# sapeirone/EgoPack

Hardware: AMD Instinct MI355X
Metric: clip-seqs/sec training, AR+LTA+PNR multi-task (higher is better)
Workload: dtype bf16; 1 GPU; MTL pre-train AR+LTA+PNR (BASELINE config 3): per GPU B=64 seqs/task x T=32 nodes, 3x1536-d Omnivore-shaped features, H=1024, TRN hidden 1024 (dropout 0.5), depth 3, k=1, Adam; graph mode, fused backbone pass; global_batch=192, parallelism=dp1, trainable_params=25003272, capture=one graph, input=resident in HBM before the timed region, master_weights=f32, mode=bf16, activations=bf16

## Files before the change

### egopack_amd/csrc/gemm.hip

```cpp
#include <type_traits>

#include "common.h"

namespace egk {

typedef __attribute__((ext_vector_type(4))) float f32x4;
typedef __attribute__((ext_vector_type(8))) __bf16 bf16x8;
typedef unsigned short bf16_t;

constexpr int BM = 128, BN = 128, ROWB = 128;
constexpr int NTHREADS = 256;

constexpr int MAXSRC = 6;
struct GemmArgs {
    int M, N;
    int nsrc;
    int K[MAXSRC];
    const void* A[MAXSRC];
    const void* B[MAXSRC];
    long long lda[MAXSRC], ldb[MAXSRC];
    int a_vec, b_vec;
    void* C;
    long long ldc;
    int c_vec, c_bf16;
// ... 13 lines not shown
    int st_mode, st_nseg;
    const int* st_seg_ptr;
    double* st_ws;
    const void* st_x;
    long long st_ldx;
    const float* st_stats;
    const float* st_w;
    const float* st_b;
    float st_slope;
};

__device__ __forceinline__ void tile_of_virtual(const GemmArgs& g, int v, int& z, int& tm, int& tn) {
    const int tiles = g.tiles_m * g.tiles_n;
    z = v / tiles;
    const int t = v - z * tiles;
    const int gsz = g.group_m * g.tiles_n;
    const int grp = t / gsz, first = grp * g.group_m;
    const int rows = min(g.group_m, g.tiles_m - first);
    const int rr = t - grp * gsz;
    tm = first + rr % rows;
    tn = rr / rows;
}
__device__ __forceinline__ void tile_of(const GemmArgs& g, int bid, int& z, int& tm, int& tn) {
    const int tiles = g.tiles_m * g.tiles_n, nwg = tiles * g.splitk;
    const int xcd = bid & 7, q = nwg >> 3, r = nwg & 7;
    const int v = (xcd < r ? xcd * (q + 1) : r * (q + 1) + (xcd - r) * q) + (bid >> 3);
    z = v / tiles;
    const int t = v - z * tiles;
    const int gsz = g.group_m * g.tiles_n;
    const int grp = t / gsz, first = grp * g.group_m;
    const int rows = min(g.group_m, g.tiles_m - first);
    const int rr = t - grp * gsz;
    tm = first + rr % rows;
    tn = rr / rows;
}

template <int KT>
__device__ __forceinline__ void source_of(const GemmArgs& g, int t, int& src, int& tt) {
    src = 0;
    tt = t;
    while (src + 1 < g.nsrc) {
        const int n = (g.K[src] + KT - 1) / KT;
        if (tt < n) break;
        tt -= n;
        ++src;
    }
}
__device__ __forceinline__ int total_tiles(const GemmArgs& g, int KT) {
    int n = 0;
    for (int s = 0; s < g.nsrc; ++s) n += (g.K[s] + KT - 1) / KT;
    return n;
}

__device__ __forceinline__ int lds_off(int row, int chunk) { return row * ROWB + ((chunk ^ ((row >> 1) & 7)) << 4); }

__device__ __forceinline__ uint4 pack8(const float* f) {
    bf16x8 v;
#pragma unroll
    for (int i = 0; i < 8; ++i) v[i] = (__bf16)f[i];
    return __builtin_bit_cast(uint4, v);
}
__device__ __forceinline__ float bf16_to_f32(bf16_t h) { return __uint_as_float((unsigned)h << 16); }
__device__ __forceinline__ bf16_t f32_to_bf16(float f) { return __builtin_bit_cast(bf16_t, (__bf16)f); }


template <bool BF16C, typename T>
__device__ __forceinline__ void load_rowmajor(const T* __restrict__ base, long long ld, int rows_total, int row0, int k0,
                                              int klim, bool vec, uint4 (&out)[8]) {
    constexpr int CE = BF16C ? 8 : 4;
    const int tid = threadIdx.x;
#pragma unroll
    for (int i = 0; i < 4; ++i) {
        const int id = tid + NTHREADS * i;
        const int r = id >> 3, c = id & 7;
        const int grow = row0 + r, gk = k0 + c * CE;
        const bool row_ok = grow < rows_total;
        const T* p = base + (long long)grow * ld + gk;
        if constexpr (sizeof(T) == 2) {
            if (row_ok && vec && gk + 8 <= klim) out[i] = *reinterpret_cast<const uint4*>(p);
            else {
                unsigned w[4] = {0, 0, 0, 0};
#pragma unroll
                for (int j = 0; j < 8; ++j)
                    if (row_ok && gk + j < klim) w[j >> 1] |= (unsigned)p[j] << (16 * (j & 1));
                out[i] = make_uint4(w[0], w[1], w[2], w[3]);
            }
        } else {
            float f[8];
            if (row_ok && vec && gk + CE <= klim) {
                const float4 v0 = *reinterpret_cast<const float4*>(p);
                f[0] = v0.x; f[1] = v0.y; f[2] = v0.z; f[3] = v0.w;
                if constexpr (BF16C) {
                    const float4 v1 = *reinterpret_cast<const float4*>(p + 4);
                    f[4] = v1.x; f[5] = v1.y; f[6] = v1.z; f[7] = v1.w;
                }
            } else {
#pragma unroll
                for (int j = 0; j < CE; ++j) f[j] = (row_ok && gk + j < klim) ? p[j] : 0.0f;
            }
            if constexpr (BF16C) out[i] = pack8(f);
            else out[i] = make_uint4(__float_as_uint(f[0]), __float_as_uint(f[1]), __float_as_uint(f[2]), __float_as_uint(f[3]));
        }
    }
}

template <bool BF16C>
// ... 445 lines not shown
        const int piece = (first + i) & 15, sub_row0 = row0 + ((first + i) >> 4) * 128;
        if constexpr (TR) {
            const int k = piece * 4 + (lane >> 4);
            const int c = (lane & 15) ^ (2 * (k & 3) + 8 * ((k >> 3) & 1));
            int col = sub_row0 + c * 8;
            if (col + 8 > ld) col = 0;
            p[i] = base + (long long)(k0 + k) * ld + col;
        } else {
            const int r = piece * 8 + (lane >> 3);
            const int c = (lane & 7) ^ ((r >> 1) & 7);
            p[i] = base + (long long)min(sub_row0 + r, rows_total - 1) * ld + k0 + c * 8;
        }
    }
    step = (TR ? 64 * ld : 64) * tiles_per_step;
}
template <int NP, int OFF = 0, int TOT = NP>
__device__ __forceinline__ void cursor_issue(const bf16_t* (&pp)[TOT], long long step, unsigned char* img, int first) {
    const bf16_t** p = pp + OFF;
#pragma unroll
    for (int i = 0; i < NP; ++i) {
        __builtin_amdgcn_global_load_lds((glb_void_t*)p[i], (lds_void_t*)(img + (first + i) * 1024), 16, 0, 0);
        p[i] += step;
    }
}
template <bool TR, int NP>
struct OperandCursor {
    const bf16_t* p[NP];
    long long step;
    __device__ __forceinline__ void init(const bf16_t* __restrict__ base, long long ld, int rows_total, int row0, int k0,
                                         int first, int lane, int tiles_per_step) {
        cursor_init<TR, NP, 0, NP>(p, step, base, ld, rows_total, row0, k0, first, lane, tiles_per_step);
    }
    __device__ __forceinline__ void issue(unsigned char* img, int first) { cursor_issue<NP, 0, NP>(p, step, img, first); }
};

typedef _Float16 f16x8 __attribute__((ext_vector_type(8)));
template <bool F16>
__device__ __forceinline__ f32x4 mfma16(const uint4& b, const uint4& a, const f32x4& c) {
    if constexpr (F16) return __builtin_amdgcn_mfma_f32_16x16x32_f16(__builtin_bit_cast(f16x8, b), __builtin_bit_cast(f16x8, a), c, 0, 0, 0);
    else return __builtin_amdgcn_mfma_f32_16x16x32_bf16(__builtin_bit_cast(bf16x8, b), __builtin_bit_cast(bf16x8, a), c, 0, 0, 0);
}

template <int NSTAGE, bool TRA, bool TRB, int KG, int MB, int NI = 4, bool VIRT = false, bool F16 = false, int LW = 0>
__device__ __forceinline__ void gemm_pipe_body(const GemmArgs& g, const int bid) {
    static_assert(KG == 1 || MB == 1, "wave groups and the tall tile are alternatives");
    static_assert(NI == 4 || ((NI == 3 || NI == 2) && !TRA && ((MB == 1 && (KG == 1 || NI == 2)) || (MB == 2 && KG == 1 && NI == 3))),
                  "96- / 64-row tiles: row-major A; two wave groups with 64-row tiles only; the tall 8-wave tile with NI = 3");
    constexpr int IMG = 16384, IMG_A = NI == 4 ? MB * IMG : MB * NI * 4096, STAGE = IMG_A + IMG;
    constexpr int NPB = 4 / MB;
    constexpr int LOADS = NI + NPB;
    constexpr int WG = 4 * MB;
    extern __shared__ __attribute__((aligned(16))) unsigned char lds[];
    constexpr int KT = 64;
#ifdef EGK_GEMM_STAMPS
    const unsigned long long ps_entry = __builtin_amdgcn_s_memtime(), ps_rentry = __builtin_amdgcn_s_memrealtime();
    unsigned long long ps_first = 0;
#endif

    int z, tm, tn;
    if constexpr (VIRT) tile_of_virtual(g, bid, z, tm, tn);
    else tile_of(g, bid, z, tm, tn);
    const int m0 = tm * (32 * NI * MB), n0 = tn * BN;
    const int nkt = total_tiles(g, KT);
    const int per = (nkt + g.splitk - 1) / g.splitk;
    const int t_begin = z * per, t_end = min(nkt, t_begin + per);

    const int tid = threadIdx.x, lane = tid & 63;
    const int wall = __builtin_amdgcn_readfirstlane(tid >> 6);
    const int grp = KG == 1 ? 0 : (wall / WG);
    const int w = wall % WG;
    const int wm = w >> 1, wn = w & 1;
    const int lr = lane & 15, lg = lane >> 4;
    unsigned char* ring = lds + grp * (NSTAGE * STAGE);

    const int nt_all = t_end - t_begin;
    const int nt = nt_all > grp ? (nt_all - grp + KG - 1) / KG : 0;
    const int rounds = (nt_all + KG - 1) / KG;

    OperandCursor<TRA, NI> ca;
    OperandCursor<TRB, NPB> cb;
    int cur_src = -1;
    auto issue = [&](int i, int stage) {
        const int t = t_begin + grp + KG * i;
        int src, tt;
        source_of<KT>(g, t, src, tt);
        if (src != cur_src) {
            const int k0 = tt * KT;
            ca.init((const bf16_t*)g.A[src], g.lda[src], g.M, m0, k0, w * NI, lane, KG);
            cb.init((const bf16_t*)g.B[src], g.ldb[src], g.N, n0, k0, w * NPB, lane, KG);
            cur_src = src;
        }
        unsigned char* sbase = ring + stage * STAGE;
        ca.issue(sbase, w * NI);
        cb.issue(sbase + IMG_A, w * NPB);
    };

    if constexpr (LW > 0) {
        static_assert(KG == 1 && (WG * NI) % LW == 0 && (WG * NPB) % LW == 0, "loader waves: one wave group, pieces divisible among the loaders");
        if (wall >= WG) {
            constexpr int PA = WG * NI / LW, PB = WG * NPB / LW;
            const int L = wall - WG;
            OperandCursor<TRA, PA> la;
            OperandCursor<TRB, PB> lb;
            int lsrc = -1;
            auto lissue = [&](int i, int stage) {
                const int t = t_begin + i;
                int src, tt;
                source_of<KT>(g, t, src, tt);
                if (src != lsrc) {
                    const int k0 = tt * KT;
                    la.init((const bf16_t*)g.A[src], g.lda[src], g.M, m0, k0, L * PA, lane, 1);
                    lb.init((const bf16_t*)g.B[src], g.ldb[src], g.N, n0, k0, L * PB, lane, 1);
                    lsrc = src;
                }
                unsigned char* sbase = ring + stage * STAGE;
                la.issue(sbase, L * PA);
                lb.issue(sbase + IMG_A, L * PB);
            };
#pragma unroll
            for (int p = 0; p < NSTAGE - 1; ++p)
                if (p < nt) lissue(p, p);
            for (int it = 0; it < rounds; ++it) {
                const int later = min(NSTAGE - 2, nt - 1 - it);
                if (later >= 2) asm volatile("s_waitcnt vmcnt(%0)" ::"n"(2 * (PA + PB)) : "memory");
                else if (later == 1) asm volatile("s_waitcnt vmcnt(%0)" ::"n"(PA + PB) : "memory");
                else asm volatile("s_waitcnt vmcnt(0)" ::: "memory");
                __builtin_amdgcn_s_barrier();
                if (it + NSTAGE - 1 < nt) lissue(it + NSTAGE - 1, (it + NSTAGE - 1) % NSTAGE);
            }
            return;
        }
    }

    f32x4 acc[NI][4];
#pragma unroll
    for (int i = 0; i < NI; ++i)
#pragma unroll
        for (int j = 0; j < 4; ++j) acc[i][j] = f32x4{0.f, 0.f, 0.f, 0.f};

    const unsigned lds_base = (unsigned)(size_t)(lds_void_t*)ring;
    const unsigned rm_sw = (unsigned)((lg ^ ((lr >> 1) & 7)) << 4);
    const unsigned a_rm = (unsigned)((wm * 16 * NI + lr) * ROWB) + rm_sw;
    const unsigned b_rm = (unsigned)((wn * 64 + lr) * ROWB) + rm_sw;
    const int tq = (lane & 15) >> 2, tp = lane & 3;
    const unsigned tr_row = (unsigned)((8 * lg + tq) * 256 + (tp & 1) * 8);
    const unsigned tr_f = (unsigned)(2 * tq + 8 * (lg & 1));
    unsigned a_tr[4], b_tr[4];
#pragma unroll
    for (int i = 0; i < 4; ++i) {
        a_tr[i] = (unsigned)((wm >> 1) * IMG) + tr_row + ((((unsigned)((wm & 1) * 8 + 2 * i + (tp >> 1))) ^ tr_f) << 4);
        b_tr[i] = tr_row + ((((unsigned)(wn * 8 + 2 * i + (tp >> 1))) ^ tr_f) << 4);
    }

    const bool do_bias = TRA && g.dbias != nullptr && tn == 0;
    float bsum[8] = {0.f, 0.f, 0.f, 0.f, 0.f, 0.f, 0.f, 0.f};
    const int bcc = tid & 15, bkg = (tid & 255) >> 4;
    const int bsub = MB == 2 ? (tid >> 8) : 0;

    uint4 a0[4], a1[4], b0[4], b1[4];
    if constexpr (LW == 0) {
#pragma unroll
        for (int p = 0; p < NSTAGE - 1; ++p)
            if (p < nt) issue(p, p);
    }
    for (int it = 0; it < rounds; ++it) {
        if constexpr (LW == 0) {
            const int later = min(NSTAGE - 2, nt - 1 - it);
            if (later >= 3) asm volatile("s_waitcnt vmcnt(%0)" ::"n"(3 * LOADS) : "memory");
            else if (later == 2) asm volatile("s_waitcnt vmcnt(%0)" ::"n"(2 * LOADS) : "memory");
            else if (later == 1) asm volatile("s_waitcnt vmcnt(%0)" ::"n"(LOADS) : "memory");
            else asm volatile("s_waitcnt vmcnt(0)" ::: "memory");
        }
        __builtin_amdgcn_s_barrier();
#ifdef EGK_GEMM_STAMPS
        if (it == 0) ps_first = __builtin_amdgcn_s_memtime();
#endif
        const unsigned stA = lds_base + (it % NSTAGE) * STAGE, stB = stA + IMG_A;
        if constexpr (LW == 0) {
            if (it + NSTAGE - 1 < nt) issue(it + NSTAGE - 1, (it + NSTAGE - 1) % NSTAGE);
        }
        if (KG > 1 && it >= nt) continue;

        uint4 bz[4];
        if constexpr (TRA) {
            if (do_bias) {
#pragma unroll
                for (int r = 0; r < 4; ++r) {
                    const int k = bkg * 4 + r;
                    const unsigned ad = stA + (unsigned)(bsub * IMG + k * 256 + ((bcc ^ (2 * (k & 3) + 8 * ((k >> 3) & 1))) << 4));
                    asm volatile("ds_read_b128 %0, %1" : "=v"(bz[r]) : "v"(ad));
                }
            }
        }
        if constexpr (TRA) {
#pragma unroll
            for (int i = 0; i < 4; ++i) {
                const unsigned ad = stA + a_tr[i];
                uint2 lo, hi;
                asm volatile("ds_read_b64_tr_b16 %0, %1" : "=v"(lo) : "v"(ad));
                asm volatile("ds_read_b64_tr_b16 %0, %1 offset:1024" : "=v"(hi) : "v"(ad));
                a0[i] = make_uint4(lo.x, lo.y, hi.x, hi.y);
            }
        } else {
#pragma unroll
            for (int i = 0; i < NI; ++i) asm volatile("ds_read_b128 %0, %1 offset:%2" : "=v"(a0[i]) : "v"(stA + a_rm), "n"(i * 2048));
        }
        if constexpr (TRB) {
#pragma unroll
            for (int j = 0; j < 4; ++j) {
                const unsigned ad = stB + b_tr[j];
                uint2 lo, hi;
                asm volatile("ds_read_b64_tr_b16 %0, %1" : "=v"(lo) : "v"(ad));
                asm volatile("ds_read_b64_tr_b16 %0, %1 offset:1024" : "=v"(hi) : "v"(ad));
                b0[j] = make_uint4(lo.x, lo.y, hi.x, hi.y);
            }
        } else {
#pragma unroll
            for (int j = 0; j < 4; ++j) asm volatile("ds_read_b128 %0, %1 offset:%2" : "=v"(b0[j]) : "v"(stB + b_rm), "n"(j * 2048));
        }
        if constexpr (TRA) {
#pragma unroll
            for (int i = 0; i < 4; ++i) {
                const unsigned ad = stA + a_tr[i];
                uint2 lo, hi;
                asm volatile("ds_read_b64_tr_b16 %0, %1 offset:8192" : "=v"(lo) : "v"(ad));
                asm volatile("ds_read_b64_tr_b16 %0, %1 offset:9216" : "=v"(hi) : "v"(ad));
                a1[i] = make_uint4(lo.x, lo.y, hi.x, hi.y);
            }
        } else {
#pragma unroll
            for (int i = 0; i < NI; ++i)
                asm volatile("ds_read_b128 %0, %1 offset:%2" : "=v"(a1[i]) : "v"((stA + a_rm) ^ 64u), "n"(i * 2048));
        }
        if constexpr (TRB) {
#pragma unroll
            for (int j = 0; j < 4; ++j) {
                const unsigned ad = stB + b_tr[j];
                uint2 lo, hi;
                asm volatile("ds_read_b64_tr_b16 %0, %1 offset:8192" : "=v"(lo) : "v"(ad));
                asm volatile("ds_read_b64_tr_b16 %0, %1 offset:9216" : "=v"(hi) : "v"(ad));
                b1[j] = make_uint4(lo.x, lo.y, hi.x, hi.y);
            }
        } else {
#pragma unroll
            for (int j = 0; j < 4; ++j)
                asm volatile("ds_read_b128 %0, %1 offset:%2" : "=v"(b1[j]) : "v"((stB + b_rm) ^ 64u), "n"(j * 2048));
        }
        constexpr int R1 = ((TRA ? 8 : NI) + (TRB ? 8 : 4)) > 15 ? 15 : ((TRA ? 8 : NI) + (TRB ? 8 : 4));
        asm volatile("s_waitcnt lgkmcnt(%0)" ::"n"(R1) : "memory");
        __builtin_amdgcn_sched_barrier(0);
#pragma unroll
        for (int i = 0; i < NI; ++i)
#pragma unroll
            for (int j = 0; j < 4; ++j)
                acc[i][j] = mfma16<F16>(b0[j], a0[i], acc[i][j]);
        asm volatile("s_waitcnt lgkmcnt(0)" ::: "memory");
        __builtin_amdgcn_sched_barrier(0);
#pragma unroll
        for (int i = 0; i < NI; ++i)
#pragma unroll
            for (int j = 0; j < 4; ++j)
                acc[i][j] = mfma16<F16>(b1[j], a1[i], acc[i][j]);
        if constexpr (TRA) {
            if (do_bias) {
#pragma unroll
                for (int r = 0; r < 4; ++r) {
                    const unsigned wv[4] = {bz[r].x, bz[r].y, bz[r].z, bz[r].w};
#pragma unroll
                    for (int e = 0; e < 4; ++e) {
                        bsum[2 * e] += __uint_as_float(wv[e] << 16);
                        bsum[2 * e + 1] += __uint_as_float(wv[e] & 0xffff0000u);
                    }
                }
            }
        }
    }
#ifdef EGK_GEMM_STAMPS
    const unsigned long long ps_loop = __builtin_amdgcn_s_memtime();
#endif
    if constexpr (TRA) {
        if (g.dbias != nullptr && tn == 0) {
            __syncthreads();
            float* red = reinterpret_cast<float*>(lds);
            const int slot = MB == 2 ? bsub : grp;
#pragma unroll
            for (int e = 0; e < 8; ++e) red[(slot * 16 + bkg) * 128 + bcc * 8 + e] = bsum[e];
            __syncthreads();
            if (tid < 128 * MB && m0 + tid < g.M) {
                const int q0 = MB == 2 ? (tid >> 7) * 16 : 0, nq = MB == 2 ? 16 : 16 * KG;
                float t = 0.f;
                for (int q = 0; q < nq; ++q) t += red[(q0 + q) * 128 + (tid & 127)];
                if (g.splitk > 1) g.ws_bias[(long long)z * g.M + m0 + tid] = t;
                else g.dbias[m0 + tid] += t;
            }
            __syncthreads();
        }
    }
    if constexpr (KG == 1) {
        if constexpr (MB == 1) {
            if (epilogue_rows_ok(g)) gemm_epilogue_rows<NI>(g, acc, lds, m0, n0, wm, wn, lr, lg, z, tid, tm * g.tiles_n + tn);
            else gemm_epilogue<NI, 4>(g, acc, m0, n0, wm * 16 * NI, wn * 64, lr, lg, z);
        } else if constexpr (NI == 3) {
            static_assert(NSTAGE * STAGE >= 192 * 512 + 256, "the rows epilogue stages the whole tile (+ the wave partials) in the ring");
            if (epilogue_rows_ok(g)) gemm_epilogue_rows<NI, true, 2>(g, acc, lds, m0, n0, wm, wn, lr, lg, z, tid, tm * g.tiles_n + tn);
            else gemm_epilogue<NI, 4>(g, acc, m0, n0, wm * 16 * NI, wn * 64, lr, lg, z);
        } else {
            gemm_epilogue<NI, 4>(g, acc, m0, n0, wm * 16 * NI, wn * 64, lr, lg, z);
        }
    } else if constexpr (NI == 4 || NI == 2) {
        constexpr int HF = NI / 2;
        __syncthreads();
        f32x4* xch = reinterpret_cast<f32x4*>(lds);
        f32x4* mine_out = xch + ((grp * 4 + w) * (HF * 4)) * 64 + lane;
        const f32x4* theirs = xch + (((1 - grp) * 4 + w) * (HF * 4)) * 64 + lane;
        f32x4 half[HF][4];
// ... 108 lines not shown


template <bool TR, int FIRST, int S, int CNT = 4>
__device__ __forceinline__ void read_frags4(uint4 (&dst)[4], unsigned st, unsigned rm, const unsigned* tr) {
    if constexpr (TR) {
#pragma unroll
        for (int i = 0; i < CNT; ++i) {
            const unsigned ad = st + tr[FIRST + i];
            uint2 lo, hi;
            asm volatile("ds_read_b64_tr_b16 %0, %1 offset:%2" : "=v"(lo) : "v"(ad), "n"(S * 8192));
            asm volatile("ds_read_b64_tr_b16 %0, %1 offset:%2" : "=v"(hi) : "v"(ad), "n"(S * 8192 + 1024));
            dst[i] = make_uint4(lo.x, lo.y, hi.x, hi.y);
        }
    } else {
        const unsigned ad = S ? ((st + rm) ^ 64u) : (st + rm);
#pragma unroll
        for (int i = 0; i < CNT; ++i) asm volatile("ds_read_b128 %0, %1 offset:%2" : "=v"(dst[i]) : "v"(ad), "n"((FIRST + i) * 2048));
    }
}
template <int NI, int CNT = 4>
__device__ __forceinline__ void mfma_4x4(f32x4 (&acc)[NI][4], int i0, const uint4 (&a)[4], const uint4 (&b)[4]) {
#pragma unroll
    for (int i = 0; i < CNT; ++i)
#pragma unroll
        for (int j = 0; j < 4; ++j)
            acc[i0 + i][j] = __builtin_amdgcn_mfma_f32_16x16x32_bf16(__builtin_bit_cast(bf16x8, b[j]), __builtin_bit_cast(bf16x8, a[i]),
                                                                     acc[i0 + i][j], 0, 0, 0);
}

template <bool TRA, bool TRB, int DMA_NBE = 8, int NI = 8>
__global__ __launch_bounds__(512) void gemm_big_kernel(const GemmArgs g) {
    static_assert(NI == 8 || (NI == 6 && !TRA), "192-row tiles: row-major A");
    constexpr int IMG = 16384, IMG_OP = 2 * IMG, STAGE = 2 * IMG_OP, KT = 64, HF = NI / 2;
    extern __shared__ __attribute__((aligned(16))) unsigned char lds[];

    int z, tm, tn;
    tile_of(g, blockIdx.x, z, tm, tn);
    const int m0 = tm * (32 * NI), n0 = tn * 256;
    const int nkt = total_tiles(g, KT);
    const int per = (nkt + g.splitk - 1) / g.splitk;
    const int t_begin = z * per, t_end = min(nkt, t_begin + per);
    const int nt = t_end - t_begin;

    const int tid = threadIdx.x, lane = tid & 63;
    const int w = __builtin_amdgcn_readfirstlane(tid >> 6);
    const int wm = w >> 2, wn = w & 3;
    const int lr = lane & 15, lg = lane >> 4;

    constexpr int NBE = DMA_NBE;
    const bool early = w < 4;
    unsigned voffA[2], voffB[2];
    const char *baseA = nullptr, *baseB = nullptr;
    long long lda_b = 0, ldb_b = 0;
    int cur_src = -1;
    auto lane_off = [&](bool tr, long long ld_bytes, int state) -> unsigned {
        if (tr) return (unsigned)((lane >> 4) * ld_bytes + ((((lane & 15) ^ (2 * ((lane >> 4) & 3) + 8 * state))) << 4));
        return (unsigned)((lane >> 3) * ld_bytes + (((lane & 7) ^ ((state << 2) | ((lane >> 4) & 3))) << 4));
    };
    auto aim = [&](int i) {
        const int t = t_begin + i;
        int src, tt;
        source_of<KT>(g, t, src, tt);
        if (src != cur_src) {
            const long long k0 = (long long)tt * KT;
            lda_b = g.lda[src] * 2; ldb_b = g.ldb[src] * 2;
            baseA = (const char*)g.A[src] + (TRA ? k0 * lda_b + (long long)m0 * 2 : (long long)m0 * lda_b + k0 * 2);
            baseB = (const char*)g.B[src] + (TRB ? k0 * ldb_b + (long long)n0 * 2 : (long long)n0 * ldb_b + k0 * 2);
#pragma unroll
            for (int x = 0; x < 2; ++x) {
                voffA[x] = lane_off(TRA, lda_b, x);
                voffB[x] = lane_off(TRB, ldb_b, x);
            }
            cur_src = src;
        }
    };
    auto issue_pieces = [&](auto trc, auto nc, const char* base, long long ld_bytes, const unsigned (&voff)[2], int first,
                            unsigned char* img) {
        constexpr bool TR = decltype(trc)::value;
        constexpr int N = decltype(nc)::value;
#pragma unroll
        for (int i = 0; i < N; ++i) {
            const int q = first + i;
            const long long off = TR ? (long long)(4 * (q & 15)) * ld_bytes + (q >> 4) * 256 : (long long)(8 * q) * ld_bytes;
            const unsigned v = voff[TR ? ((i >> 1) & 1) : (i & 1)];
            __builtin_amdgcn_global_load_lds((glb_void_t*)(base + off + v), (lds_void_t*)(img + q * 1024), 16, 0, 0);
        }
    };
    using std::integral_constant;
    auto advance = [&]() {
        baseA += TRA ? KT * lda_b : KT * 2;
        baseB += TRB ? KT * ldb_b : KT * 2;
    };
    auto issue_early = [&](unsigned char* stage) {
        issue_pieces(integral_constant<bool, TRA>{}, integral_constant<int, NI>{}, baseA, lda_b, voffA, w * NI, stage);
        issue_pieces(integral_constant<bool, TRB>{}, integral_constant<int, NBE>{}, baseB, ldb_b, voffB, w * NBE, stage + IMG_OP);
    };
    auto issue_late = [&](unsigned char* stage) {
        if constexpr (NBE < 8)
            issue_pieces(integral_constant<bool, TRB>{}, integral_constant<int, 8 - NBE>{}, baseB, ldb_b, voffB,
                         4 * NBE + (w - 4) * (8 - NBE), stage + IMG_OP);
    };

    f32x4 acc[NI][4];
#pragma unroll
    for (int i = 0; i < NI; ++i)
#pragma unroll
        for (int j = 0; j < 4; ++j) acc[i][j] = f32x4{0.f, 0.f, 0.f, 0.f};

    const unsigned lds_base = (unsigned)(size_t)(lds_void_t*)lds;
    const unsigned rm_sw = (unsigned)((lg ^ ((lr >> 1) & 7)) << 4);
    const unsigned a_rm = (unsigned)((wm * 16 * NI + lr) * ROWB) + rm_sw;
    const unsigned b_rm = (unsigned)((wn >> 1) * IMG + ((wn & 1) * 64 + lr) * ROWB) + rm_sw;
    const int tq = (lane & 15) >> 2, tp = lane & 3;
    const unsigned tr_row = (unsigned)((8 * lg + tq) * 256 + (tp & 1) * 8);
    const unsigned tr_f = (unsigned)(2 * tq + 8 * (lg & 1));
    unsigned a_tr[NI], b_tr[4];
#pragma unroll
    for (int i = 0; i < NI; ++i) a_tr[i] = (unsigned)(wm * IMG) + tr_row + ((((unsigned)(2 * i + (tp >> 1))) ^ tr_f) << 4);
#pragma unroll
    for (int j = 0; j < 4; ++j)
        b_tr[j] = (unsigned)((wn >> 1) * IMG) + tr_row + ((((unsigned)((wn & 1) * 8 + 2 * j + (tp >> 1))) ^ tr_f) << 4);

#ifdef EGK_GEMM_STAMPS
    unsigned long long st_wait = 0, st_issue = 0, st_head = 0, st_body = 0;
    const unsigned long long st_begin = __builtin_amdgcn_s_memtime(), st_rbegin = __builtin_amdgcn_s_memrealtime();
#define EGK_STAMP(var) const unsigned long long var = __builtin_amdgcn_s_memtime()
#else
#define EGK_STAMP(var)
#endif
    if (nt > 0) {
        aim(0);
        if (early) issue_early(lds);
        else issue_late(lds);
        advance();
    }
    for (int it = 0; it < nt; ++it) {
        EGK_STAMP(s0);
        asm volatile("s_waitcnt vmcnt(0)" ::: "memory");
        __builtin_amdgcn_s_barrier();
        EGK_STAMP(s1);
        const bool more = it + 1 < nt;
        unsigned char* nxt = lds + ((it + 1) & 1) * STAGE;
        if (more) aim(it + 1);
        if (more && early) issue_early(nxt);
        EGK_STAMP(s2);

        const unsigned stA = lds_base + (it & 1) * STAGE, stB = stA + IMG_OP;
        uint4 b0[4], b1[4], alo[4], ahi[4];
        constexpr int NA = TRA ? 8 : HF, NB = TRB ? 8 : 4;
        read_frags4<TRB, 0, 0>(b0, stB, b_rm, b_tr);
        read_frags4<TRA, 0, 0, HF>(alo, stA, a_rm, a_tr);
        read_frags4<TRA, HF, 0, HF>(ahi, stA, a_rm, a_tr);
        asm volatile("s_waitcnt lgkmcnt(%0)" ::"n"(NA) : "memory");
        __builtin_amdgcn_sched_barrier(0);
        EGK_STAMP(s3);
        mfma_4x4<NI, HF>(acc, 0, alo, b0);
        __builtin_amdgcn_sched_barrier(0);
        read_frags4<TRB, 0, 1>(b1, stB, b_rm, b_tr);
        read_frags4<TRA, 0, 1, HF>(alo, stA, a_rm, a_tr);
        asm volatile("s_waitcnt lgkmcnt(%0)" ::"n"(NA + NB > 15 ? 15 : NA + NB) : "memory");
        __builtin_amdgcn_sched_barrier(0);
        mfma_4x4<NI, HF>(acc, HF, ahi, b0);
        __builtin_amdgcn_sched_barrier(0);
        if (more && !early) issue_late(nxt);
        if (more) advance();
        read_frags4<TRA, HF, 1, HF>(ahi, stA, a_rm, a_tr);
        asm volatile("s_waitcnt lgkmcnt(%0)" ::"n"(NA) : "memory");
        __builtin_amdgcn_sched_barrier(0);
        mfma_4x4<NI, HF>(acc, 0, alo, b1);
        asm volatile("s_waitcnt lgkmcnt(0)" ::: "memory");
        __builtin_amdgcn_sched_barrier(0);
        mfma_4x4<NI, HF>(acc, HF, ahi, b1);
#ifdef EGK_GEMM_STAMPS
        __builtin_amdgcn_sched_barrier(0);
        EGK_STAMP(s4);
        st_wait += s1 - s0; st_issue += s2 - s1; st_head += s3 - s2; st_body += s4 - s3;
#endif
    }
#ifdef EGK_GEMM_STAMPS
    if (g.ws_bias != nullptr && lane == 0) {
        unsigned long long* o = reinterpret_cast<unsigned long long*>(g.ws_bias) + ((long long)blockIdx.x * 8 + w) * 8;
        o[0] = st_wait; o[1] = st_issue; o[2] = st_head; o[3] = st_body;
        o[4] = __builtin_amdgcn_s_memtime() - st_begin; o[5] = __builtin_amdgcn_s_memrealtime() - st_rbegin; o[6] = nt;
    }
#endif
#undef EGK_STAMP
    gemm_epilogue<NI, 4>(g, acc, m0, n0, wm * 16 * NI, wn * 64, lr, lg, z);
}

template <bool TR, int NP>
__device__ __forceinline__ void cursor32_init(const float* (&p)[NP], long long& step, const float* __restrict__ base, long long ld,
                                              int rows_total, int row0, int k0, int first, int lane) {
#pragma unroll
    for (int i = 0; i < NP; ++i) {
        const int piece = first + i;
        if constexpr (TR) {
            const int k = piece * 2 + (lane >> 5);
            const int c = (lane & 31) ^ (((k >> 2) & 3) << 2);
            int col = row0 + c * 4;
            if (col + 4 > ld) col = 0;
            p[i] = base + (long long)(k0 + k) * ld + col;
        } else {
            const int r = piece * 8 + (lane >> 3);
            const int c = (lane & 7) ^ ((r >> 1) & 7);
            p[i] = base + (long long)min(row0 + r, rows_total - 1) * ld + k0 + c * 4;
        }
    }
    step = TR ? 32 * ld : 32;
}

template <bool TR, int S_, int NF>
__device__ __forceinline__ void read_step32(float (&f)[NF][4], unsigned st, unsigned rm, const unsigned (&tr)[4]) {
    if constexpr (TR) {
#pragma unroll
        for (int q = 0; q < 4; ++q)
#pragma unroll
            for (int i = 0; i < NF; ++i)
                asm volatile("ds_read_b32 %0, %1 offset:%2" : "=v"(f[i][q]) : "v"(st + tr[i]), "n"((16 * S_ + q) * 512));
    } else {
#pragma unroll
        for (int i = 0; i < NF; ++i) {
            f32x4 v;
            asm volatile("ds_read_b128 %0, %1 offset:%2" : "=v"(v) : "v"(S_ ? ((st + rm) ^ 64u) : (st + rm)), "n"(i * 2048));
            f[i][0] = v[0]; f[i][1] = v[1]; f[i][2] = v[2]; f[i][3] = v[3];
        }
    }
}

template <bool TRA, bool TRB, int NI = 4, bool VIRT = false>
__device__ __forceinline__ void gemm_pipe_f32_body(const GemmArgs& g, const int bid) {
    static_assert(NI == 4 || (NI == 3 && !TRA), "96-row tiles: row-major A");
    constexpr int IMG = 16384, IMG_A = NI * 4096, STAGE = IMG_A + IMG, KT = 32;
    extern __shared__ __attribute__((aligned(16))) unsigned char lds[];
    int z, tm, tn;
    if constexpr (VIRT) tile_of_virtual(g, bid, z, tm, tn);
    else tile_of(g, bid, z, tm, tn);
    const int m0 = tm * (32 * NI), n0 = tn * BN;
    const int nkt = total_tiles(g, KT);
    const int per = (nkt + g.splitk - 1) / g.splitk;
    const int t_begin = z * per, t_end = min(nkt, t_begin + per);
    const int nt = t_end - t_begin;

    const int tid = threadIdx.x, lane = tid & 63;
    const int w = __builtin_amdgcn_readfirstlane(tid >> 6);
    const int wm = w >> 1, wn = w & 1;
    const int lr = lane & 15, lg = lane >> 4;

    const float* pa[NI];
    const float* pb[4];
    long long sa = 0, sb = 0;
    int cur_src = -1;
    auto issue = [&](int i, int stage) {
        int src, tt;
        source_of<KT>(g, t_begin + i, src, tt);
        if (src != cur_src) {
            cursor32_init<TRA, NI>(pa, sa, (const float*)g.A[src], g.lda[src], g.M, m0, tt * KT, w * NI, lane);
            cursor32_init<TRB, 4>(pb, sb, (const float*)g.B[src], g.ldb[src], g.N, n0, tt * KT, w * 4, lane);
            cur_src = src;
        }
        unsigned char* sbase = lds + stage * STAGE;
#pragma unroll
        for (int q = 0; q < NI; ++q) {
            __builtin_amdgcn_global_load_lds((glb_void_t*)pa[q], (lds_void_t*)(sbase + (w * NI + q) * 1024), 16, 0, 0);
            pa[q] += sa;
        }
#pragma unroll
        for (int q = 0; q < 4; ++q) {
            __builtin_amdgcn_global_load_lds((glb_void_t*)pb[q], (lds_void_t*)(sbase + IMG_A + (w * 4 + q) * 1024), 16, 0, 0);
            pb[q] += sb;
        }
    };

    f32x4 acc[NI][4];
#pragma unroll
    for (int i = 0; i < NI; ++i)
#pragma unroll
        for (int j = 0; j < 4; ++j) acc[i][j] = f32x4{0.f, 0.f, 0.f, 0.f};

    const unsigned lds_base = (unsigned)(size_t)(lds_void_t*)lds;
    const unsigned rm_sw = (unsigned)((lg ^ ((lr >> 1) & 7)) << 4);
    const unsigned a_rm = (unsigned)((wm * 16 * NI + lr) * ROWB) + rm_sw, b_rm = (unsigned)((wn * 64 + lr) * ROWB) + rm_sw;
    unsigned a_tr[4], b_tr[4];
#pragma unroll
    for (int i = 0; i < 4; ++i) {
        a_tr[i] = (unsigned)(4 * lg * 512 + ((((wm * 16 + i * 4 + (lr >> 2)) ^ (lg << 2))) << 4) + (lr & 3) * 4);
        b_tr[i] = (unsigned)(4 * lg * 512 + ((((wn * 16 + i * 4 + (lr >> 2)) ^ (lg << 2))) << 4) + (lr & 3) * 4);
    }

    auto mfma_step = [&](const float (&fa)[NI][4], const float (&fb)[4][4]) {
#pragma unroll
        for (int q = 0; q < 4; ++q)
#pragma unroll
            for (int i = 0; i < NI; ++i)
#pragma unroll
                for (int j = 0; j < 4; ++j) acc[i][j] = __builtin_amdgcn_mfma_f32_16x16x4f32(fb[j][q], fa[i][q], acc[i][j], 0, 0, 0);
    };
    const bool do_bias = TRA && g.dbias != nullptr && tn == 0;
    float bsum[4] = {0.f, 0.f, 0.f, 0.f};
    const int bcc = tid & 31, bkg = tid >> 5;
    if (nt > 0) issue(0, 0);
    for (int it = 0; it < nt; ++it) {
        asm volatile("s_waitcnt vmcnt(0)" ::: "memory");
        __builtin_amdgcn_s_barrier();
        if (it + 1 < nt) issue(it + 1, (it + 1) & 1);
        const unsigned stA = lds_base + (it & 1) * STAGE, stB = stA + IMG_A;
        float a0[NI][4], b0[4][4], a1[NI][4], b1[4][4];
        f32x4 bz[4];
        if constexpr (TRA) {
            if (do_bias) {
#pragma unroll
                for (int r = 0; r < 4; ++r) {
                    const int k = bkg * 4 + r;
                    const unsigned ad = stA + (unsigned)(k * 512 + ((bcc ^ (((k >> 2) & 3) << 2)) << 4));
                    asm volatile("ds_read_b128 %0, %1" : "=v"(bz[r]) : "v"(ad));
                }
            }
        }
        read_step32<TRA, 0, NI>(a0, stA, a_rm, a_tr);
        read_step32<TRB, 0, 4>(b0, stB, b_rm, b_tr);
        asm volatile("s_waitcnt lgkmcnt(0)" ::: "memory");
        __builtin_amdgcn_sched_barrier(0);
        read_step32<TRA, 1, NI>(a1, stA, a_rm, a_tr);
        read_step32<TRB, 1, 4>(b1, stB, b_rm, b_tr);
        mfma_step(a0, b0);
        asm volatile("s_waitcnt lgkmcnt(0)" ::: "memory");
        __builtin_amdgcn_sched_barrier(0);
        mfma_step(a1, b1);
        if constexpr (TRA) {
            if (do_bias) {
#pragma unroll
                for (int r = 0; r < 4; ++r)
#pragma unroll
                    for (int e = 0; e < 4; ++e) bsum[e] += bz[r][e];
            }
        }
    }
    if constexpr (TRA) {
        if (g.dbias != nullptr && tn == 0) {
            __syncthreads();
            float* red = reinterpret_cast<float*>(lds);
#pragma unroll
            for (int e = 0; e < 4; ++e) red[bkg * 128 + bcc * 4 + e] = bsum[e];
            __syncthreads();
            if (tid < 128 && m0 + tid < g.M) {
                float t = 0.f;
                for (int q = 0; q < 8; ++q) t += red[q * 128 + tid];
                if (g.splitk > 1) g.ws_bias[(long long)z * g.M + m0 + tid] = t;
                else g.dbias[m0 + tid] += t;
            }
            __syncthreads();
        }
    }
    if (epilogue_rows_ok(g)) gemm_epilogue_rows<NI>(g, acc, lds, m0, n0, wm, wn, lr, lg, z, tid, tm * g.tiles_n + tn);
    else gemm_epilogue<NI, 4>(g, acc, m0, n0, wm * 16 * NI, wn * 64, lr, lg, z);
}

template <bool TRA, bool TRB, int NI = 4>
__global__ __launch_bounds__(NTHREADS) void gemm_pipe_f32_kernel(const GemmArgs g) {
    gemm_pipe_f32_body<TRA, TRB, NI, false>(g, blockIdx.x);
}

template <bool TRA, bool TRB>
__global__ __launch_bounds__(NTHREADS) void gemm_pipe_f32_group_kernel(const GemmGroup gg) {
    const int lin = blockIdx.x, xcd = lin & 7, slot = lin >> 3;
    const int q = gg.total >> 3, r = gg.total & 7;
    if (slot >= q + (xcd < r ? 1 : 0)) return;
    int v = (xcd < r ? xcd * (q + 1) : r * (q + 1) + (xcd - r) * q) + slot;
    int pi = 0;
    for (; pi + 1 < gg.count; ++pi) {
        const int t = gg.p[pi].tiles_m * gg.p[pi].tiles_n;
        if (v < t) break;
        v -= t;
    }
    gemm_pipe_f32_body<TRA, TRB, 4, true>(gg.p[pi], v);
}

__global__ __launch_bounds__(256) void gemm_splitk_reduce(const GemmArgs g) {
// ... 642 lines not shown
```

Measured before the change: 148,600 clip-seqs/s.

## Interleave LDS transpose reads with MFMA rows and walk K sources incrementally

For GEMMs with both operands transposed, the LDS fragment reads are split so that each row of MFMAs waits only on the reads it needs (fine-grained lgkmcnt). This lets the second half-step's transpose reads overlap the first half's matrix math. The per-tile source lookup loop is replaced by an incremental SourceWalk cursor in all pipelines. Extra sched_barriers are placed around the waitcnts so the compiler cannot move LDS reads across them. The hand-tuned wait counts are fragile and could stall or race if they are miscounted.

```diff
diff --git a/egopack_amd/csrc/gemm.hip b/egopack_amd/csrc/gemm.hip
--- a/egopack_amd/csrc/gemm.hip
+++ b/egopack_amd/csrc/gemm.hip
@@ -89,6 +89,34 @@
     return n;
 }
 
+template <int KT, int STRIDE = 1>
+struct SourceWalk {
+    int src, tt, n, run, left;
+    __device__ __forceinline__ void start(const GemmArgs& g, int t0) {
+        src = 0;
+        tt = t0;
+        n = (g.K[0] + KT - 1) / KT;
+        run = 0;
+        left = 0;
+    }
+    __device__ __forceinline__ bool next(const GemmArgs& g) {
+        if (left > 0) {
+            --left;
+            return false;
+        }
+        tt += STRIDE * run;
+        const int nsrc = g.nsrc;
+        while (src + 1 < nsrc && tt >= n) {
+            tt -= n;
+            ++src;
+            n = (g.K[src] + KT - 1) / KT;
+        }
+        run = src + 1 < nsrc ? (n - tt + STRIDE - 1) / STRIDE : 0x7fffffff / STRIDE;
+        left = run - 1;
+        return true;
+    }
+};
+
 __device__ __forceinline__ int lds_off(int row, int chunk) { return row * ROWB + ((chunk ^ ((row >> 1) & 7)) << 4); }
 
 __device__ __forceinline__ uint4 pack8(const float* f) {
@@ -640,6 +668,7 @@
     constexpr int WG = 4 * MB;
     extern __shared__ __attribute__((aligned(16))) unsigned char lds[];
     constexpr int KT = 64;
+    constexpr bool FINE = TRA && TRB && KG == 1 && LW == 0;
 #ifdef EGK_GEMM_STAMPS
     const unsigned long long ps_entry = __builtin_amdgcn_s_memtime(), ps_rentry = __builtin_amdgcn_s_memrealtime();
     unsigned long long ps_first = 0;
@@ -667,16 +696,13 @@
 
     OperandCursor<TRA, NI> ca;
     OperandCursor<TRB, NPB> cb;
-    int cur_src = -1;
-    auto issue = [&](int i, int stage) {
-        const int t = t_begin + grp + KG * i;
-        int src, tt;
-        source_of<KT>(g, t, src, tt);
-        if (src != cur_src) {
-            const int k0 = tt * KT;
+    SourceWalk<KT, KG> walk;
+    walk.start(g, t_begin + grp);
+    auto issue = [&](int stage) {
+        if (walk.next(g)) {
+            const int src = walk.src, k0 = walk.tt * KT;
             ca.init((const bf16_t*)g.A[src], g.lda[src], g.M, m0, k0, w * NI, lane, KG);
             cb.init((const bf16_t*)g.B[src], g.ldb[src], g.N, n0, k0, w * NPB, lane, KG);
-            cur_src = src;
         }
         unsigned char* sbase = ring + stage * STAGE;
         ca.issue(sbase, w * NI);
@@ -690,16 +716,13 @@
             const int L = wall - WG;
             OperandCursor<TRA, PA> la;
             OperandCursor<TRB, PB> lb;
-            int lsrc = -1;
-            auto lissue = [&](int i, int stage) {
-                const int t = t_begin + i;
-                int src, tt;
-                source_of<KT>(g, t, src, tt);
-                if (src != lsrc) {
-                    const int k0 = tt * KT;
+            SourceWalk<KT> lwalk;
+            lwalk.start(g, t_begin);
+            auto lissue = [&](int stage) {
+                if (lwalk.next(g)) {
+                    const int src = lwalk.src, k0 = lwalk.tt * KT;
                     la.init((const bf16_t*)g.A[src], g.lda[src], g.M, m0, k0, L * PA, lane, 1);
                     lb.init((const bf16_t*)g.B[src], g.ldb[src], g.N, n0, k0, L * PB, lane, 1);
-                    lsrc = src;
                 }
                 unsigned char* sbase = ring + stage * STAGE;
                 la.issue(sbase, L * PA);
@@ -707,14 +730,14 @@
             };
 #pragma unroll
             for (int p = 0; p < NSTAGE - 1; ++p)
-                if (p < nt) lissue(p, p);
+                if (p < nt) lissue(p);
             for (int it = 0; it < rounds; ++it) {
                 const int later = min(NSTAGE - 2, nt - 1 - it);
                 if (later >= 2) asm volatile("s_waitcnt vmcnt(%0)" ::"n"(2 * (PA + PB)) : "memory");
                 else if (later == 1) asm volatile("s_waitcnt vmcnt(%0)" ::"n"(PA + PB) : "memory");
                 else asm volatile("s_waitcnt vmcnt(0)" ::: "memory");
                 __builtin_amdgcn_s_barrier();
-                if (it + NSTAGE - 1 < nt) lissue(it + NSTAGE - 1, (it + NSTAGE - 1) % NSTAGE);
+                if (it + NSTAGE - 1 < nt) lissue((it + NSTAGE - 1) % NSTAGE);
             }
             return;
         }
@@ -749,7 +772,7 @@
     if constexpr (LW == 0) {
 #pragma unroll
         for (int p = 0; p < NSTAGE - 1; ++p)
-            if (p < nt) issue(p, p);
+            if (p < nt) issue(p);
     }
     for (int it = 0; it < rounds; ++it) {
         if constexpr (LW == 0) {
@@ -765,7 +788,7 @@
 #endif
         const unsigned stA = lds_base + (it % NSTAGE) * STAGE, stB = stA + IMG_A;
         if constexpr (LW == 0) {
-            if (it + NSTAGE - 1 < nt) issue(it + NSTAGE - 1, (it + NSTAGE - 1) % NSTAGE);
+            if (it + NSTAGE - 1 < nt) issue((it + NSTAGE - 1) % NSTAGE);
         }
         if (KG > 1 && it >= nt) continue;
 
@@ -780,75 +803,112 @@
                 }
             }
         }
-        if constexpr (TRA) {
-#pragma unroll
-            for (int i = 0; i < 4; ++i) {
-                const unsigned ad = stA + a_tr[i];
+        if constexpr (FINE) {
+            using std::integral_constant;
+            auto read_tr = [&](uint4& dst, unsigned ad, auto off) {
+                constexpr int OFFS = decltype(off)::value;
                 uint2 lo, hi;
-                asm volatile("ds_read_b64_tr_b16 %0, %1" : "=v"(lo) : "v"(ad));
-                asm volatile("ds_read_b64_tr_b16 %0, %1 offset:1024" : "=v"(hi) : "v"(ad));
-                a0[i] = make_uint4(lo.x, lo.y, hi.x, hi.y);
-            }
+                asm volatile("ds_read_b64_tr_b16 %0, %1 offset:%2" : "=v"(lo) : "v"(ad), "n"(OFFS));
+                asm volatile("ds_read_b64_tr_b16 %0, %1 offset:%2" : "=v"(hi) : "v"(ad), "n"(OFFS + 1024));
+                dst = make_uint4(lo.x, lo.y, hi.x, hi.y);
+            };
+            auto row = [&](const uint4 (&a)[4], const uint4 (&b)[4], int i, auto cnt) {
+                __builtin_amdgcn_sched_barrier(0);
+                asm volatile("s_waitcnt lgkmcnt(%0)" ::"n"(decltype(cnt)::value) : "memory");
+                __builtin_amdgcn_sched_barrier(0);
+#pragma unroll
+                for (int j = 0; j < 4; ++j) acc[i][j] = mfma16<F16>(b[j], a[i], acc[i][j]);
+                __builtin_amdgcn_sched_barrier(0);
+            };
+#pragma unroll
+            for (int j = 0; j < 4; ++j) read_tr(b0[j], stB + b_tr[j], integral_constant<int, 0>{});
+#pragma unroll
+            for (int i = 0; i < 4; ++i) read_tr(a0[i], stA + a_tr[i], integral_constant<int, 0>{});
+            row(a0, b0, 0, integral_constant<int, 6>{});
+            row(a0, b0, 1, integral_constant<int, 4>{});
+#pragma unroll
+            for (int j = 0; j < 4; ++j) read_tr(b1[j], stB + b_tr[j], integral_constant<int, 8192>{});
+            row(a0, b0, 2, integral_constant<int, 10>{});
+            row(a0, b0, 3, integral_constant<int, 8>{});
+#pragma unroll
+            for (int i = 0; i < 4; ++i) read_tr(a1[i], stA + a_tr[i], integral_constant<int, 8192>{});
+            row(a1, b1, 0, integral_constant<int, 6>{});
+            row(a1, b1, 1, integral_constant<int, 4>{});
+            row(a1, b1, 2, integral_constant<int, 2>{});
+            row(a1, b1, 3, integral_constant<int, 0>{});
         } else {
-#pragma unroll
-            for (int i = 0; i < NI; ++i) asm volatile("ds_read_b128 %0, %1 offset:%2" : "=v"(a0[i]) : "v"(stA + a_rm), "n"(i * 2048));
-        }
-        if constexpr (TRB) {
-#pragma unroll
-            for (int j = 0; j < 4; ++j) {
-                const unsigned ad = stB + b_tr[j];
-                uint2 lo, hi;
-                asm volatile("ds_read_b64_tr_b16 %0, %1" : "=v"(lo) : "v"(ad));
-                asm volatile("ds_read_b64_tr_b16 %0, %1 offset:1024" : "=v"(hi) : "v"(ad));
-                b0[j] = make_uint4(lo.x, lo.y, hi.x, hi.y);
-            }
-        } else {
-#pragma unroll
-            for (int j = 0; j < 4; ++j) asm volatile("ds_read_b128 %0, %1 offset:%2" : "=v"(b0[j]) : "v"(stB + b_rm), "n"(j * 2048));
-        }
-        if constexpr (TRA) {
-#pragma unroll
-            for (int i = 0; i < 4; ++i) {
-                const unsigned ad = stA + a_tr[i];
-                uint2 lo, hi;
-                asm volatile("ds_read_b64_tr_b16 %0, %1 offset:8192" : "=v"(lo) : "v"(ad));
-                asm volatile("ds_read_b64_tr_b16 %0, %1 offset:9216" : "=v"(hi) : "v"(ad));
-                a1[i] = make_uint4(lo.x, lo.y, hi.x, hi.y);
-            }
-        } else {
+            if constexpr (TRA) {
+#pragma unroll
+                for (int i = 0; i < 4; ++i) {
+                    const unsigned ad = stA + a_tr[i];
+                    uint2 lo, hi;
+                    asm volatile("ds_read_b64_tr_b16 %0, %1" : "=v"(lo) : "v"(ad));
+                    asm volatile("ds_read_b64_tr_b16 %0, %1 offset:1024" : "=v"(hi) : "v"(ad));
+                    a0[i] = make_uint4(lo.x, lo.y, hi.x, hi.y);
+                }
+            } else {
+#pragma unroll
+                for (int i = 0; i < NI; ++i) asm volatile("ds_read_b128 %0, %1 offset:%2" : "=v"(a0[i]) : "v"(stA + a_rm), "n"(i * 2048));
+            }
+            if constexpr (TRB) {
+#pragma unroll
+                for (int j = 0; j < 4; ++j) {
+                    const unsigned ad = stB + b_tr[j];
+                    uint2 lo, hi;
+                    asm volatile("ds_read_b64_tr_b16 %0, %1" : "=v"(lo) : "v"(ad));
+                    asm volatile("ds_read_b64_tr_b16 %0, %1 offset:1024" : "=v"(hi) : "v"(ad));
+                    b0[j] = make_uint4(lo.x, lo.y, hi.x, hi.y);
+                }
+            } else {
+#pragma unroll
+                for (int j = 0; j < 4; ++j) asm volatile("ds_read_b128 %0, %1 offset:%2" : "=v"(b0[j]) : "v"(stB + b_rm), "n"(j * 2048));
+            }
+            if constexpr (TRA) {
+#pragma unroll
+                for (int i = 0; i < 4; ++i) {
+                    const unsigned ad = stA + a_tr[i];
+                    uint2 lo, hi;
+                    asm volatile("ds_read_b64_tr_b16 %0, %1 offset:8192" : "=v"(lo) : "v"(ad));
+                    asm volatile("ds_read_b64_tr_b16 %0, %1 offset:9216" : "=v"(hi) : "v"(ad));
+                    a1[i] = make_uint4(lo.x, lo.y, hi.x, hi.y);
+                }
+            } else {
+#pragma unroll
+                for (int i = 0; i < NI; ++i)
+                    asm volatile("ds_read_b128 %0, %1 offset:%2" : "=v"(a1[i]) : "v"((stA + a_rm) ^ 64u), "n"(i * 2048));
+            }
+            if constexpr (TRB) {
+#pragma unroll
+                for (int j = 0; j < 4; ++j) {
+                    const unsigned ad = stB + b_tr[j];
+                    uint2 lo, hi;
+                    asm volatile("ds_read_b64_tr_b16 %0, %1 offset:8192" : "=v"(lo) : "v"(ad));
+                    asm volatile("ds_read_b64_tr_b16 %0, %1 offset:9216" : "=v"(hi) : "v"(ad));
+                    b1[j] = make_uint4(lo.x, lo.y, hi.x, hi.y);
+                }
+            } else {
+#pragma unroll
+                for (int j = 0; j < 4; ++j)
+                    asm volatile("ds_read_b128 %0, %1 offset:%2" : "=v"(b1[j]) : "v"((stB + b_rm) ^ 64u), "n"(j * 2048));
+            }
+            constexpr int R1 = ((TRA ? 8 : NI) + (TRB ? 8 : 4)) > 15 ? 15 : ((TRA ? 8 : NI) + (TRB ? 8 : 4));
+            __builtin_amdgcn_sched_barrier(0);
+            asm volatile("s_waitcnt lgkmcnt(%0)" ::"n"(R1) : "memory");
+            __builtin_amdgcn_sched_barrier(0);
 #pragma unroll
             for (int i = 0; i < NI; ++i)
-                asm volatile("ds_read_b128 %0, %1 offset:%2" : "=v"(a1[i]) : "v"((stA + a_rm) ^ 64u), "n"(i * 2048));
-        }
-        if constexpr (TRB) {
-#pragma unroll
-            for (int j = 0; j < 4; ++j) {
-                const unsigned ad = stB + b_tr[j];
-                uint2 lo, hi;
-                asm volatile("ds_read_b64_tr_b16 %0, %1 offset:8192" : "=v"(lo) : "v"(ad));
-                asm volatile("ds_read_b64_tr_b16 %0, %1 offset:9216" : "=v"(hi) : "v"(ad));
-                b1[j] = make_uint4(lo.x, lo.y, hi.x, hi.y);
-            }
-        } else {
-#pragma unroll
-            for (int j = 0; j < 4; ++j)
-                asm volatile("ds_read_b128 %0, %1 offset:%2" : "=v"(b1[j]) : "v"((stB + b_rm) ^ 64u), "n"(j * 2048));
-        }
-        constexpr int R1 = ((TRA ? 8 : NI) + (TRB ? 8 : 4)) > 15 ? 15 : ((TRA ? 8 : NI) + (TRB ? 8 : 4));
-        asm volatile("s_waitcnt lgkmcnt(%0)" ::"n"(R1) : "memory");
-        __builtin_amdgcn_sched_barrier(0);
-#pragma unroll
-        for (int i = 0; i < NI; ++i)
-#pragma unroll
-            for (int j = 0; j < 4; ++j)
-                acc[i][j] = mfma16<F16>(b0[j], a0[i], acc[i][j]);
-        asm volatile("s_waitcnt lgkmcnt(0)" ::: "memory");
-        __builtin_amdgcn_sched_barrier(0);
-#pragma unroll
-        for (int i = 0; i < NI; ++i)
-#pragma unroll
-            for (int j = 0; j < 4; ++j)
-                acc[i][j] = mfma16<F16>(b1[j], a1[i], acc[i][j]);
+#pragma unroll
+                for (int j = 0; j < 4; ++j)
+                    acc[i][j] = mfma16<F16>(b0[j], a0[i], acc[i][j]);
+            __builtin_amdgcn_sched_barrier(0);
+            asm volatile("s_waitcnt lgkmcnt(0)" ::: "memory");
+            __builtin_amdgcn_sched_barrier(0);
+#pragma unroll
+            for (int i = 0; i < NI; ++i)
+#pragma unroll
+                for (int j = 0; j < 4; ++j)
+                    acc[i][j] = mfma16<F16>(b1[j], a1[i], acc[i][j]);
+        }
         if constexpr (TRA) {
             if (do_bias) {
 #pragma unroll
@@ -1063,17 +1123,16 @@
     unsigned voffA[2], voffB[2];
     const char *baseA = nullptr, *baseB = nullptr;
     long long lda_b = 0, ldb_b = 0;
-    int cur_src = -1;
+    SourceWalk<KT> walk;
+    walk.start(g, t_begin);
     auto lane_off = [&](bool tr, long long ld_bytes, int state) -> unsigned {
         if (tr) return (unsigned)((lane >> 4) * ld_bytes + ((((lane & 15) ^ (2 * ((lane >> 4) & 3) + 8 * state))) << 4));
         return (unsigned)((lane >> 3) * ld_bytes + (((lane & 7) ^ ((state << 2) | ((lane >> 4) & 3))) << 4));
     };
-    auto aim = [&](int i) {
-        const int t = t_begin + i;
-        int src, tt;
-        source_of<KT>(g, t, src, tt);
-        if (src != cur_src) {
-            const long long k0 = (long long)tt * KT;
+    auto aim = [&]() {
+        if (walk.next(g)) {
+            const int src = walk.src;
+            const long long k0 = (long long)walk.tt * KT;
             lda_b = g.lda[src] * 2; ldb_b = g.ldb[src] * 2;
             baseA = (const char*)g.A[src] + (TRA ? k0 * lda_b + (long long)m0 * 2 : (long long)m0 * lda_b + k0 * 2);
             baseB = (const char*)g.B[src] + (TRB ? k0 * ldb_b + (long long)n0 * 2 : (long long)n0 * ldb_b + k0 * 2);
@@ -1082,7 +1141,6 @@
                 voffA[x] = lane_off(TRA, lda_b, x);
                 voffB[x] = lane_off(TRB, ldb_b, x);
             }
-            cur_src = src;
         }
     };
     auto issue_pieces = [&](auto trc, auto nc, const char* base, long long ld_bytes, const unsigned (&voff)[2], int first,
@@ -1140,7 +1198,7 @@
 #define EGK_STAMP(var)
 #endif
     if (nt > 0) {
-        aim(0);
+        aim();
         if (early) issue_early(lds);
         else issue_late(lds);
         advance();
@@ -1152,7 +1210,7 @@
         EGK_STAMP(s1);
         const bool more = it + 1 < nt;
         unsigned char* nxt = lds + ((it + 1) & 1) * STAGE;
-        if (more) aim(it + 1);
+        if (more) aim();
         if (more && early) issue_early(nxt);
         EGK_STAMP(s2);
 
@@ -1162,6 +1220,7 @@
         read_frags4<TRB, 0, 0>(b0, stB, b_rm, b_tr);
         read_frags4<TRA, 0, 0, HF>(alo, stA, a_rm, a_tr);
         read_frags4<TRA, HF, 0, HF>(ahi, stA, a_rm, a_tr);
+        __builtin_amdgcn_sched_barrier(0);
         asm volatile("s_waitcnt lgkmcnt(%0)" ::"n"(NA) : "memory");
         __builtin_amdgcn_sched_barrier(0);
         EGK_STAMP(s3);
@@ -1169,6 +1228,7 @@
         __builtin_amdgcn_sched_barrier(0);
         read_frags4<TRB, 0, 1>(b1, stB, b_rm, b_tr);
         read_frags4<TRA, 0, 1, HF>(alo, stA, a_rm, a_tr);
+        __builtin_amdgcn_sched_barrier(0);
         asm volatile("s_waitcnt lgkmcnt(%0)" ::"n"(NA + NB > 15 ? 15 : NA + NB) : "memory");
         __builtin_amdgcn_sched_barrier(0);
         mfma_4x4<NI, HF>(acc, HF, ahi, b0);
@@ -1176,9 +1236,11 @@
         if (more && !early) issue_late(nxt);
         if (more) advance();
         read_frags4<TRA, HF, 1, HF>(ahi, stA, a_rm, a_tr);
+        __builtin_amdgcn_sched_barrier(0);
         asm volatile("s_waitcnt lgkmcnt(%0)" ::"n"(NA) : "memory");
         __builtin_amdgcn_sched_barrier(0);
         mfma_4x4<NI, HF>(acc, 0, alo, b1);
+        __builtin_amdgcn_sched_barrier(0);
         asm volatile("s_waitcnt lgkmcnt(0)" ::: "memory");
         __builtin_amdgcn_sched_barrier(0);
         mfma_4x4<NI, HF>(acc, HF, ahi, b1);
@@ -1260,14 +1322,13 @@
     const float* pa[NI];
     const float* pb[4];
     long long sa = 0, sb = 0;
-    int cur_src = -1;
-    auto issue = [&](int i, int stage) {
-        int src, tt;
-        source_of<KT>(g, t_begin + i, src, tt);
-        if (src != cur_src) {
+    SourceWalk<KT> walk;
+    walk.start(g, t_begin);
+    auto issue = [&](int stage) {
+        if (walk.next(g)) {
+            const int src = walk.src, tt = walk.tt;
             cursor32_init<TRA, NI>(pa, sa, (const float*)g.A[src], g.lda[src], g.M, m0, tt * KT, w * NI, lane);
             cursor32_init<TRB, 4>(pb, sb, (const float*)g.B[src], g.ldb[src], g.N, n0, tt * KT, w * 4, lane);
-            cur_src = src;
         }
         unsigned char* sbase = lds + stage * STAGE;
 #pragma unroll
@@ -1309,11 +1370,11 @@
     const bool do_bias = TRA && g.dbias != nullptr && tn == 0;
     float bsum[4] = {0.f, 0.f, 0.f, 0.f};
     const int bcc = tid & 31, bkg = tid >> 5;
-    if (nt > 0) issue(0, 0);
+    if (nt > 0) issue(0);
     for (int it = 0; it < nt; ++it) {
         asm volatile("s_waitcnt vmcnt(0)" ::: "memory");
         __builtin_amdgcn_s_barrier();
-        if (it + 1 < nt) issue(it + 1, (it + 1) & 1);
+        if (it + 1 < nt) issue((it + 1) & 1);
         const unsigned stA = lds_base + (it & 1) * STAGE, stB = stA + IMG_A;
         float a0[NI][4], b0[4][4], a1[NI][4], b1[4][4];
         f32x4 bz[4];
@@ -1329,11 +1390,13 @@
         }
         read_step32<TRA, 0, NI>(a0, stA, a_rm, a_tr);
         read_step32<TRB, 0, 4>(b0, stB, b_rm, b_tr);
+        __builtin_amdgcn_sched_barrier(0);
         asm volatile("s_waitcnt lgkmcnt(0)" ::: "memory");
         __builtin_amdgcn_sched_barrier(0);
         read_step32<TRA, 1, NI>(a1, stA, a_rm, a_tr);
         read_step32<TRB, 1, 4>(b1, stB, b_rm, b_tr);
         mfma_step(a0, b0);
+        __builtin_amdgcn_sched_barrier(0);
         asm volatile("s_waitcnt lgkmcnt(0)" ::: "memory");
         __builtin_amdgcn_sched_barrier(0);
         mfma_step(a1, b1);
```

Result: no change. 148,700 clip-seqs/s, median of 3 (+0.1%).
